# goalheart/ionic-mpnn

Measured on AMD Instinct MI355X. Metric: molecule-graph pairs/sec (fwd), batch 4096 per MI355X, higher is better.
Workload: dtype f32 (bf16x9 emulation)

## Files before the change

### ionic_mpnn_amd/csrc/encoder_typed.hip

```cpp
#include "encoder_device.h"
#include "encoder_layout.h"
#include "kernel_device.h"

namespace impnn {
namespace enc {

namespace {

constexpr int kOffUpd = 0;
constexpr int off_h(bool x3) { return kOffUpd + (x3 ? kXUpdLds : kTUpdLds); }
constexpr int kTHSBig3 = 32;
constexpr int off_msg(bool x3, int hs = kTHS) { return off_h(x3) + kRCap * hs; }
constexpr int off_rec(bool x3, int ecap, int hs = kTHS) { return off_msg(x3, hs) + tmsg_floats(ecap); }
constexpr size_t lds_fixed_bytes(bool x3, int Vb, int ecap, int hs = kTHS) {
  return sizeof(float) * (size_t)off_rec(x3, ecap, hs) + trec_lds_bytes(Vb, ecap);
}
static_assert(lds_fixed_bytes(true, kTVbMax, kTECap) <= 160 * 1024 && lds_fixed_bytes(false, kTVbMax, kTECapBig) <= 160 * 1024 &&
                  lds_fixed_bytes(true, kTVbMax, kTECapBig, kTHSBig3) <= 160 * 1024,
              "LDS budget");

typedef bf16x8_t bf16x8;
struct B3 {
  bf16x8 p0, p1, p2;
};
__device__ __forceinline__ B3 split8x3(f32x4 a, f32x4 b) {
  union {
    bf16x8 v;
    unsigned u[4];
  } q0, q1, q2;
  split_pair(a[0], a[1], q0.u[0], q1.u[0], q2.u[0]);
  split_pair(a[2], a[3], q0.u[1], q1.u[1], q2.u[1]);
  split_pair(b[0], b[1], q0.u[2], q1.u[2], q2.u[2]);
  split_pair(b[2], b[3], q0.u[3], q1.u[3], q2.u[3]);
  B3 r;
  r.p0 = q0.v;
  r.p1 = q1.v;
  r.p2 = q2.v;
  return r;
}
__device__ __forceinline__ void mma9x2(f32x4& c0, f32x4& c1, const __bf16* blk0, const __bf16* blk1, int lane, const B3& b) {
  const bf16x8 a00 = *reinterpret_cast<const bf16x8*>(blk0 + lane * 8);
  const bf16x8 a01 = *reinterpret_cast<const bf16x8*>(blk0 + 512 + lane * 8);
  const bf16x8 a02 = *reinterpret_cast<const bf16x8*>(blk0 + 1024 + lane * 8);
  const bf16x8 a10 = *reinterpret_cast<const bf16x8*>(blk1 + lane * 8);
  const bf16x8 a11 = *reinterpret_cast<const bf16x8*>(blk1 + 512 + lane * 8);
  const bf16x8 a12 = *reinterpret_cast<const bf16x8*>(blk1 + 1024 + lane * 8);
  c0 = mfma_bf16(a02, b.p2, c0);  c1 = mfma_bf16(a12, b.p2, c1);
  c0 = mfma_bf16(a01, b.p2, c0);  c1 = mfma_bf16(a11, b.p2, c1);
  c0 = mfma_bf16(a02, b.p1, c0);  c1 = mfma_bf16(a12, b.p1, c1);
  c0 = mfma_bf16(a00, b.p2, c0);  c1 = mfma_bf16(a10, b.p2, c1);
  c0 = mfma_bf16(a02, b.p0, c0);  c1 = mfma_bf16(a12, b.p0, c1);
  c0 = mfma_bf16(a01, b.p1, c0);  c1 = mfma_bf16(a11, b.p1, c1);
  c0 = mfma_bf16(a00, b.p1, c0);  c1 = mfma_bf16(a10, b.p1, c1);
  c0 = mfma_bf16(a01, b.p0, c0);  c1 = mfma_bf16(a11, b.p0, c1);
  c0 = mfma_bf16(a00, b.p0, c0);  c1 = mfma_bf16(a10, b.p0, c1);
}

template <int ABID>
__device__ __forceinline__ f32x4 mfma1(float a, float b, f32x4 c) {
  return __builtin_amdgcn_mfma_f32_4x4x1f32(a, b, c, 3, ABID, 0);
}

typedef float f32x2v __attribute__((ext_vector_type(2)));
typedef __attribute__((address_space(3))) void* lds_ptr_t;
__device__ __forceinline__ void glds16(const void* gsrc, const float* dst) {
  const unsigned lds_dst = __builtin_amdgcn_readfirstlane((unsigned)(uintptr_t)(lds_ptr_t)dst);
  unsigned keep;
  asm volatile("s_mov_b32 %0, m0\n\ts_mov_b32 m0, %2\n\ts_nop 0\n\tglobal_load_lds_dwordx4 %1, off\n\ts_mov_b32 m0, %0"
               : "=&s"(keep)
               : "v"(gsrc), "s"(lds_dst)
               : "memory");
}
struct Grp {
  uint4 ge;
  f32x2v aq;
};
struct Run {
  f32x4 bq[4];
  Grp first;
};

__device__ __forceinline__ void group_messages(const f32x2v aq, const f32x4 (&bq)[4], float& m01, float& m23) {
  f32x4 acc0 = {0.f, 0.f, 0.f, 0.f}, acc1 = acc0;
#ifndef IMPNN_DIAG_NO_MSG_MFMA
  acc0 = mfma1<0>(aq[0], bq[0][0], acc0);
  acc1 = mfma1<0>(aq[1], bq[0][1], acc1);
  acc0 = mfma1<1>(aq[0], bq[0][2], acc0);
  acc1 = mfma1<1>(aq[1], bq[0][3], acc1);
  acc0 = mfma1<2>(aq[0], bq[1][0], acc0);
  acc1 = mfma1<2>(aq[1], bq[1][1], acc1);
  acc0 = mfma1<3>(aq[0], bq[1][2], acc0);
  acc1 = mfma1<3>(aq[1], bq[1][3], acc1);
  acc0 = mfma1<4>(aq[0], bq[2][0], acc0);
  acc1 = mfma1<4>(aq[1], bq[2][1], acc1);
  acc0 = mfma1<5>(aq[0], bq[2][2], acc0);
  acc1 = mfma1<5>(aq[1], bq[2][3], acc1);
  acc0 = mfma1<6>(aq[0], bq[3][0], acc0);
  acc1 = mfma1<6>(aq[1], bq[3][1], acc1);
  acc0 = mfma1<7>(aq[0], bq[3][2], acc0);
  acc1 = mfma1<7>(aq[1], bq[3][3], acc1);
#else
  acc0[0] = aq[0] + bq[0][0] + bq[3][3];
  acc1[1] = aq[1] + bq[1][1] + bq[2][2];
#endif
  float x0 = acc0[0] + acc1[0], x1 = acc0[1] + acc1[1], x2 = acc0[2] + acc1[2], x3 = acc0[3] + acc1[3];
  asm volatile("s_nop 1\n\tv_permlane32_swap_b32 %0, %1\n\tv_permlane32_swap_b32 %2, %3"
               : "+v"(x0), "+v"(x1), "+v"(x2), "+v"(x3));
  m01 = x0 + x1;
  m23 = x2 + x3;
}

__global__ __launch_bounds__(256) void typed_m0_kernel(const float* tmat0, const float* atom_table, float* m0,
                                                       M0Header* hdr, int Va, int Vb, int S) {
  const int lane = threadIdx.x & 63;
  const int w = __builtin_amdgcn_readfirstlane(blockIdx.x * 4 + (threadIdx.x >> 6));
  const int nga = (Va + 4) >> 2;
  if (w < Vb * nga) {
    const int v = w / nga, a0 = 4 * (w - v * nga);
    const int kh = lane >> 5, f = lane & 31;
    const int ai = a0 + (lane & 3);
    f32x2v aq = {0.f, 0.f};
    if (ai < Va) aq = *reinterpret_cast<const f32x2v*>(atom_table + (size_t)ai * kD + 16 * kh + 2 * ((lane >> 2) & 7));
    const float* bp = tmat0 + (size_t)v * kTMatFloats + kh * 512 + f * 4;
    f32x4 bq[4];
#pragma unroll
    for (int i = 0; i < 4; ++i) bq[i] = ld4(bp + i * 128);
    float m01, m23;
    group_messages(aq, bq, m01, m23);
    float* row = m0 + (size_t)v * (Va + 1) * kD + f;
    if (a0 + kh <= Va) row[(size_t)(a0 + kh) * kD] = m01;
    if (a0 + 2 + kh <= Va) row[(size_t)(a0 + 2 + kh) * kD] = m23;
  }
  if (blockIdx.x == 0 && threadIdx.x == 0) *hdr = M0Header{kM0Magic, Va, Vb, S};
}

#ifndef IMPNN_T_PF
#define IMPNN_T_PF 0
#endif
#ifndef IMPNN_T_EARLY
#define IMPNN_T_EARLY 0
#endif
constexpr int kPfWhere = IMPNN_T_PF, kRunsEarly = IMPNN_T_EARLY;
template <int N, bool LANES>
__device__ __forceinline__ void reduce_ranks(const float* msg, const uint16_t* jdptr, int d0, int deg, int row, int q,
                                             int zero_slot, f32x4& agg0, f32x4& agg1) {
  const uint2 jd = *reinterpret_cast<const uint2*>(jdptr + d0);
  const int first[4] = {(int)(jd.x & 0xffffu), (int)(jd.x >> 16), (int)(jd.y & 0xffffu), (int)(jd.y >> 16)};
  f32x4 m0v[N], m1v[N];
#pragma unroll
  for (int j = 0; j < N; ++j) {
    const int o = tmsg_off(d0 + j < deg ? first[j] + row : zero_slot, q);
    m0v[j] = ld4(msg + o);
    m1v[j] = ld4(msg + (o ^ 16));
  }
#pragma unroll
  for (int j = 0; j < N; ++j) {
    if constexpr (LANES) {
#pragma unroll
      for (int i = 0; i < 4; ++i) {
        agg0[i] = lane1(agg0[i] + m0v[j][i]);
        agg1[i] = lane1(agg1[i] + m1v[j][i]);
      }
    } else {
      agg0 += m0v[j];
      agg1 += m1v[j];
    }
  }
}

__device__ __forceinline__ float keep1(float v) { return lane1(v); }
__device__ __forceinline__ f32x4 keep1(f32x4 v) { return v; }
template <bool LANES, class F, class... A>
__device__ __forceinline__ f32x4 quad(F f, A... a) {
  if constexpr (LANES) {
    f32x4 r;
#pragma unroll
    for (int i = 0; i < 4; ++i) r[i] = f(a[i]...);
    return r;
  } else {
    return f(a...);
  }
}

template <bool STAMPS, bool X3, int HS = kTHS>
__global__ __launch_bounds__(kThreads, kThreads / 256) void encoder_typed_kernel(TEncParams p) {
  extern __shared__ __align__(16) float smem[];
  constexpr int kUpdLds = X3 ? kXUpdLds : kTUpdLds, kUpdSlot = X3 ? kXUpdSlot : kTUpdSlot;
  constexpr int kNPf = X3 ? 3 : 2;
  float* const wupd = smem + kOffUpd;
  float* const wvec = wupd + (X3 ? kXVecFloatOff : kTVecFloatOff);
  float* const hbuf = smem + off_h(X3);
  float* const msg = smem + off_msg(X3, HS);
  const int zero_slot = p.ecap + 1;
  unsigned char* const recl = reinterpret_cast<unsigned char*>(smem + off_rec(X3, p.ecap, HS));
  const int rec_lds = p.rec_lds;
  float* const atab = reinterpret_cast<float*>(recl + rec_lds);
  const uint16_t* const r_rowdeg = reinterpret_cast<const uint16_t*>(recl + kTRecRowdeg);
  const unsigned char* const r_tilemax = recl + kTRecTilemax;
  const uint16_t* const r_moloff = reinterpret_cast<const uint16_t*>(recl + kTRecMoloff);
  const uint16_t* const r_molrows = reinterpret_cast<const uint16_t*>(recl + kTRecMolrows);
  const uint16_t* const r_poolrow = reinterpret_cast<const uint16_t*>(recl + kTRecPoolrow);
  const int32_t* const r_rowatom = reinterpret_cast<const int32_t*>(recl + kTRecRowatom);
  const uint16_t* const r_jdptr = reinterpret_cast<const uint16_t*>(recl + kTRecJdptr);
  const uint16_t* const r_runs = reinterpret_cast<const uint16_t*>(recl + trec_runs_off(p.Vb, p.ecap));
  int* const run_ctr = reinterpret_cast<int*>(recl + kTRecCounts + 8);
  const uint4* const r_grp = reinterpret_cast<const uint4*>(recl + kTRecGrp);

  const int tid = threadIdx.x, lane = tid & 63;
  const int wave = __builtin_amdgcn_readfirstlane(tid >> 6);
  const int a = lane & 15, q = lane >> 4;
  unsigned long long* stamp = STAMPS && p.stamps ? p.stamps + (size_t)blockIdx.x * 32 : nullptr;
  if (stamp && tid == 0) stamp[0] = __builtin_amdgcn_s_memtime();

  {
    const PlanHeader hd = *p.header;
    if (hd.magic != kPlanMagic || hd.kind != 1 || hd.nwg != (int)gridDim.x || hd.max_sub != p.max_sub ||
        hd.B != p.B || hd.n_ions != p.n_ions || hd.overflow != 0) {
      const float nan = __builtin_nanf("");
      for (int g = 0; g < p.n_ions; ++g)
        for (int64_t t = (int64_t)blockIdx.x * kThreads + tid; t < (int64_t)p.B * kD; t += (int64_t)gridDim.x * kThreads)
          p.pooled[g][t] = nan;
      return;
    }
  }
  const int c_begin = blockIdx.x * p.max_sub;
  const int c_end = c_begin + __builtin_amdgcn_readfirstlane(p.nsub[blockIdx.x]);
  if (c_begin >= c_end) return;

  if (p.atab_lds)
    for (int t = tid; t < (p.Va + 1) * (kTAS / 4); t += kThreads)
      st4(atab + 4 * t, t < p.Va * (kD / 4) ? ld4(p.atom_table + 4 * t) : f32x4{0.f, 0.f, 0.f, 0.f});
  if (tid < kD) msg[zero_slot * kD + tid] = 0.f;
  unsigned long long t_pro = 0, t_steps = 0, t_pool = 0, t_mark = 0, t_msg = 0;
  if (stamp && tid == 0) t_mark = __builtin_amdgcn_s_memtime();

  auto pool = [&](int M, int m0, int g) {
    float* out_g = p.pooled[g];
    for (int t0 = 0; t0 < M * 64; t0 += kThreads) {
      const int t = t0 + tid;
      const int part = t & 7, f4 = (t >> 3) & 7, m = t >> 6;
      f32x4 acc = {0.f, 0.f, 0.f, 0.f};
      if (m < M) {
        const int nr = r_molrows[m], mo = r_moloff[m];
        for (int n = part; n < nr; n += 8) {
          const int pr = r_poolrow[mo + n];
          if (pr & 0x8000) acc += ld4(hbuf + (pr & 0xff) * HS + 4 * f4);
        }
      }
#pragma unroll
      for (int i = 0; i < 4; ++i) {
        float v = acc[i];
        v += __builtin_bit_cast(float, __builtin_amdgcn_update_dpp(0, __builtin_bit_cast(int, v), 0xb1, 0xf, 0xf, true));
        v += __builtin_bit_cast(float, __builtin_amdgcn_update_dpp(0, __builtin_bit_cast(int, v), 0x4e, 0xf, 0xf, true));
        v += __builtin_bit_cast(float, __builtin_amdgcn_update_dpp(0, __builtin_bit_cast(int, v), 0x141, 0xf, 0xf, true));
        acc[i] = v;
      }
      if (m < M && part == 0) st4(out_g + (int64_t)(m0 + m) * kD + 4 * f4, acc);
    }
  };
  auto fill_h0 = [&]() {
    const int row = tid >> 2, sub = tid & 3;
    const int id = r_rowatom[row];
    f32x4 v0 = {0.f, 0.f, 0.f, 0.f}, v1 = v0;
    if ((unsigned)id < (unsigned)p.Va) {
      if (p.atab_lds) {
        v0 = ld4(atab + id * kTAS + 8 * sub);
        v1 = ld4(atab + id * kTAS + 8 * sub + 4);
      } else {
        int sb = sub;
        asm volatile("" : "+v"(sb));
        v0 = ld4(p.atom_table + (int64_t)id * kD + 8 * sb);
        v1 = ld4(p.atom_table + (int64_t)id * kD + 8 * sb + 4);
      }
    }
    st4(hbuf + row * HS + 8 * sub, v0);
    st4(hbuf + row * HS + 8 * sub + 4, v1);
  };

  if (p.S == 0) {
    for (int c = c_begin; c < c_end; ++c) {
      const unsigned char* rc = p.rec + (size_t)c * kTRecBytes;
      if (8 * tid < rec_lds) reinterpret_cast<uint2*>(recl)[tid] = reinterpret_cast<const uint2*>(rc)[tid];
      const int4 dsc = reinterpret_cast<const int4*>(p.desc)[c];
      lds_barrier();
      fill_h0();
      lds_barrier();
      pool(__builtin_amdgcn_readfirstlane(dsc.y), __builtin_amdgcn_readfirstlane(dsc.x),
           __builtin_amdgcn_readfirstlane(dsc.w) >> 16);
      lds_barrier();
    }
    return;
  }

  unsigned tabmask = 0;
  {
    const M0Header t0 = *reinterpret_cast<const M0Header*>(p.upd[0] + kUpdLds);
    if (t0.magic == kM0Magic && t0.Va == p.Va && t0.Vb == p.Vb && t0.S == p.S) tabmask |= 1u;
    if (p.n_ions > 1) {
      const M0Header t1 = *reinterpret_cast<const M0Header*>(p.upd[1] + kUpdLds);
      if (t1.magic == kM0Magic && t1.Va == p.Va && t1.Vb == p.Vb && t1.S == p.S) tabmask |= 2u;
    }
  }

  const bool rec_big = rec_lds > kTRecPart1;
  const unsigned char* rec_c = p.rec + (size_t)c_begin * kTRecBytes;
  uint2 rec_n8 = reinterpret_cast<const uint2*>(rec_c)[tid];
  uint32_t rec_n4 = rec_big ? reinterpret_cast<const uint32_t*>(rec_c + kTRecPart1)[tid] : 0u;
  int4 dsc_next = reinterpret_cast<const int4*>(p.desc)[c_begin];

  auto fetch_step0 = [&](const int4 dn, int cn) {
    const int gn = __builtin_amdgcn_readfirstlane(dn.w) >> 16;
    const float* const ug = p.upd[gn];
    static_assert(kUpdLds % 256 == 0, "whole 64-lane transfers");
    int ln = lane, wv = wave;
    asm volatile("" : "+v"(ln), "+s"(wv));
    const bool tabn = (tabmask >> gn) & 1u;
    int edges = __builtin_amdgcn_readfirstlane(dn.z);
    edges = tabn ? (edges < p.ecap ? edges : p.ecap) : 0;
    constexpr int kIt = (kTECapBig / 8 + kWaves - 1) / kWaves;
    uint32_t sw[kIt];
    if (tabn) {
      const uint32_t* const lst = p.slist + (size_t)cn * p.ecap;
#pragma unroll
      for (int i = 0; i < kIt; ++i) {
        const int sl = 8 * (wv + i * kWaves) + (ln >> 3);
        const uint32_t word = lst[sl < edges ? sl : 0];
        sw[i] = sl < edges ? word : 0u;
      }
    } else {
#pragma unroll
      for (int i = 0; i < kIt; ++i) sw[i] = 0u;
    }
    constexpr int kUIt = (kUpdLds / 256 + kWaves - 1) / kWaves;
#pragma unroll
    for (int i = 0; i < kUIt; ++i) {
      const int ub = 64 * (wv + i * kWaves);
      if (ub < kUpdLds / 4) glds16(ug + 4 * (ub + ln), wupd + 4 * ub);
    }
    static_assert(kIt == 5, "the list words are landed by name");
    asm volatile("" : "+v"(sw[0]), "+v"(sw[1]), "+v"(sw[2]), "+v"(sw[3]), "+v"(sw[4]) : : "memory");
    const float* const m0_g = p.m0[gn];
#pragma unroll
    for (int i = 0; i < kIt; ++i) {
      const int base = 8 * (wv + i * kWaves);
      if (base < edges) {
        const int sl = base + (ln >> 3);
        const unsigned type = min(sw[i] >> 24, (unsigned)p.Vb - 1u), col = min(sw[i] & kSrcIdNone, (unsigned)p.Va);
        const unsigned off = (type * (unsigned)(p.Va + 1) + col) * kD + 4u * ((ln & 7) ^ ((sl >> 1) & 7));
        glds16(m0_g + off, msg + kD * base);
      }
    }
  };
  fetch_step0(dsc_next, c_begin);

  const uint32_t* const grp_x = reinterpret_cast<const uint32_t*>(r_grp);
  const int kh = lane >> 5, f = lane & 31;
  const int boff = kh * 512 + f * 4;
  const int ysh = 8 * (lane & 3), zsh = 16 * kh;
  const int acol = 16 * kh + 2 * ((lane >> 2) & 7);

  for (int c = c_begin; c < c_end; ++c) {
    const int4 dsc = dsc_next;
    const int m0 = __builtin_amdgcn_readfirstlane(dsc.x), M = __builtin_amdgcn_readfirstlane(dsc.y);
    const int rg = __builtin_amdgcn_readfirstlane(dsc.w);
    const int R = rg & 0xffff, g = rg >> 16;
    const int ntiles = (R + 15) >> 4;
    const float* upd_g = p.upd[g];
    const float* tmat_g = p.tmat[g];
    const bool tab0 = (tabmask >> g) & 1u;
    if (8 * tid < rec_lds) reinterpret_cast<uint2*>(recl)[tid] = rec_n8;
    if (rec_big && kTRecPart1 + 4 * tid < rec_lds) reinterpret_cast<uint32_t*>(recl + kTRecPart1)[tid] = rec_n4;
    lds_barrier();
    fill_h0();
    if (tid == 0) *run_ctr = 2 * kWaves;
    asm volatile("s_waitcnt vmcnt(0) lgkmcnt(0)\n\ts_barrier" ::: "memory");
    {
      const int cn = (c + 1) < c_end ? (c + 1) : c;
      const unsigned char* rn = p.rec + (size_t)cn * kTRecBytes;
      rec_n8 = reinterpret_cast<const uint2*>(rn)[tid];
      if (rec_big) rec_n4 = reinterpret_cast<const uint32_t*>(rn + kTRecPart1)[tid];
      dsc_next = reinterpret_cast<const int4*>(p.desc)[cn];
    }
    if (stamp && tid == 0) {
      const unsigned long long t = __builtin_amdgcn_s_memtime();
      t_pro += t - t_mark;
      t_mark = t;
    }
    const int nrun = __builtin_amdgcn_readfirstlane(*reinterpret_cast<const uint16_t*>(recl + kTRecNrun));

    Run P, Q;
    int gP = 0, nP = 0, gQ = 0, nQ = 0;
    bool haveP = false, haveQ = false;
    const bool sP = wave < nrun, sQ = wave + kWaves < nrun;
    const int sgP = __builtin_amdgcn_readfirstlane(r_runs[sP ? wave : 0]);
    const int snP = __builtin_amdgcn_readfirstlane(r_runs[(sP ? wave : 0) + 1]) - sgP;
    const int sgQ = __builtin_amdgcn_readfirstlane(r_runs[sQ ? wave + kWaves : 0]);
    const int snQ = __builtin_amdgcn_readfirstlane(r_runs[(sQ ? wave + kWaves : 0) + 1]) - sgQ;
    const int soP = sP ? (__builtin_amdgcn_readfirstlane(grp_x[4 * sgP]) & 0xff) * kTMatFloats : 0;
    const int soQ = sQ ? (__builtin_amdgcn_readfirstlane(grp_x[4 * sgQ]) & 0xff) * kTMatFloats : 0;
    const int lboffP = sP ? boff : 0, lboffQ = sQ ? boff : 0;
    f32x4 pf[kNPf];
    auto fetch_pf = [&](int s_) {
#pragma unroll
      for (int i = 0; i < kNPf; ++i) pf[i] = ld4(upd_g + (int64_t)s_ * kUpdSlot + 4 * (tid + i * kThreads));
    };
    auto fetch_P = [&](int s_) {
      const float* tm = tmat_g + (size_t)s_ * p.Vb * kTMatFloats;
#pragma unroll
      for (int i = 0; i < 4; ++i) P.bq[i] = ld4(tm + soP + lboffP + i * 128);
    };
    auto fetch_Q = [&](int s_) {
      const float* tm = tmat_g + (size_t)s_ * p.Vb * kTMatFloats;
#pragma unroll
      for (int i = 0; i < 4; ++i) Q.bq[i] = ld4(tm + soQ + lboffQ + i * 128);
    };
    if (kRunsEarly >= 1) fetch_P(0);
    if (kRunsEarly >= 2) fetch_Q(0);
    if (stamp && c == c_begin && tid == 0) stamp[13] = __builtin_amdgcn_s_memtime();
    for (int s = 0; s < p.S; ++s) {
      const float* tm_s = tmat_g + (size_t)s * p.Vb * kTMatFloats;
      __builtin_amdgcn_s_setprio(2);
      const bool from_tab = tab0 && s == 0;
      if (kPfWhere == 0) {
        if (s > 0) {
          fetch_pf(s);
        } else {
#pragma unroll
          for (int i = 0; i < kNPf; ++i) pf[i] = f32x4{0.f, 0.f, 0.f, 0.f};
        }
      }
      if (!from_tab) {
        const float* const abase = hbuf + acol;
        auto load_group = [&](int e, Grp& G) {
          G.ge = r_grp[e];
          const int src = __builtin_amdgcn_ubfe(G.ge.y, ysh, 8);
          G.aq = *reinterpret_cast<const f32x2v*>(abase + src * HS);
        };
        auto compute = [&](const Grp& G, const f32x4 (&bq)[4]) {
          float m01, m23;
          group_messages(G.aq, bq, m01, m23);
          msg[__builtin_amdgcn_ubfe(G.ge.z, zsh, 16) ^ f] = m01;
          msg[__builtin_amdgcn_ubfe(G.ge.w, zsh, 16) ^ f] = m23;
        };
        auto run_type = [&](int g_, int n_, Run& Rn) {
          const int end = g_ + n_;
          Grp T;
          int e = g_;
          while (true) {
            if (e + 1 < end) load_group(e + 1, T);
            compute(Rn.first, Rn.bq);
            if (++e >= end) break;
            if (e + 1 < end) load_group(e + 1, Rn.first);
            compute(T, Rn.bq);
            if (++e >= end) break;
          }
        };
        auto fetch = [&](bool have, int r, int& g_, int& n_, Run& Rn, const float* tm) {
          const int rc = have ? r : 0;
          g_ = __builtin_amdgcn_readfirstlane(r_runs[rc]);
          n_ = __builtin_amdgcn_readfirstlane(r_runs[rc + 1]) - g_;
          const int type = have ? (__builtin_amdgcn_readfirstlane(grp_x[4 * g_]) & 0xff) : 0;
          const float* bp = tm + (size_t)type * kTMatFloats + (have ? boff : 0);
#pragma unroll
          for (int i = 0; i < 4; ++i) Rn.bq[i] = ld4(bp + i * 128);
        };
        auto next_run = [&]() {
          int r = 0;
          if (lane == 0) r = atomicAdd(run_ctr, 1);
          return __builtin_amdgcn_readfirstlane(r);
        };
        auto take = [&](int r, int& g_, int& n_, Run& Rn) {
          fetch(true, r, g_, n_, Rn, tm_s);
          load_group(g_, Rn.first);
        };
        auto landed = [](f32x4 (&b)[4]) {
          asm volatile("" : "+v"(b[0]), "+v"(b[1]), "+v"(b[2]), "+v"(b[3]) : : "memory");
        };
        if (kRunsEarly < 1) fetch_P(s);
        if (kRunsEarly < 2) fetch_Q(s);
        haveP = sP; gP = sgP; nP = snP;
        haveQ = sQ; gQ = sgQ; nQ = snQ;
        if (haveP) load_group(gP, P.first);
        if (haveQ) load_group(gQ, Q.first);
        if (haveP) {
          if (!haveQ) {
            landed(P.bq);
            run_type(gP, nP, P);
          } else {
            while (true) {
              landed(P.bq);
              run_type(gP, nP, P);
              const int rP = next_run();
              if (rP >= nrun) {
                landed(Q.bq);
                run_type(gQ, nQ, Q);
                break;
              }
              take(rP, gP, nP, P);
              landed(Q.bq);
              run_type(gQ, nQ, Q);
              const int rQ = next_run();
              if (rQ >= nrun) {
                landed(P.bq);
                run_type(gP, nP, P);
                break;
              }
              take(rQ, gQ, nQ, Q);
            }
          }
        }
        landed(P.bq);
        landed(Q.bq);
      }
      if (s > 0) {
#pragma unroll
        for (int i = 0; i < kNPf; ++i)
          if (4 * (tid + i * kThreads) < kUpdLds) st4(wupd + 4 * (tid + i * kThreads), pf[i]);
      }
      const bool mstamp = stamp && c == c_begin && s == 1;
      if (mstamp && lane == 0) stamp[16 + wave] = __builtin_amdgcn_s_memtime();
      lds_barrier();
      if (tid == 0) *run_ctr = 2 * kWaves;
      if (mstamp && tid == 0) stamp[12] = __builtin_amdgcn_s_memtime();
      if (stamp && tid == 0 && c == c_begin && s == 1) t_msg = __builtin_amdgcn_s_memtime();

      int my_tile = -1;
      {
        const int grp = wave & 3, slot = wave >> 2, q4 = ntiles >> 2, r4 = ntiles & 3;
        const int heavy = (4 - r4) * q4;
        if (grp >= r4) {
          if (slot < q4) my_tile = slot * (4 - r4) + (grp - r4);
        } else if (slot <= q4) {
          my_tile = heavy + slot * r4 + grp;
        }
      }
      const bool has_tile = my_tile >= 0 && my_tile < ntiles;
      if (has_tile) {
        const int tile = my_tile;
        const int row = tile * 16 + a;
        const int deg = r_rowdeg[row];
        const int maxdeg = __builtin_amdgcn_readfirstlane(r_tilemax[tile]);
        f32x4 h0, h1, z0, z1, r0, r1;
        [[maybe_unused]] const __bf16* const wb = reinterpret_cast<const __bf16*>(wupd);
        if constexpr (X3) {
          h0 = ld4(hbuf + row * HS + 4 * q);
          h1 = ld4(hbuf + row * HS + 16 + 4 * q);
          z0 = ld4(wvec + 0 * kD + 4 * q), z1 = ld4(wvec + 0 * kD + 16 + 4 * q);
          r0 = ld4(wvec + 1 * kD + 4 * q), r1 = ld4(wvec + 1 * kD + 16 + 4 * q);
          const B3 sh = split8x3(h0, h1);
          mma9x2(z0, z1, wb + ((0 * 2 + 0) * 2 + 0) * 1536, wb + ((0 * 2 + 1) * 2 + 0) * 1536, lane, sh);
          mma9x2(r0, r1, wb + ((1 * 2 + 0) * 2 + 0) * 1536, wb + ((1 * 2 + 1) * 2 + 0) * 1536, lane, sh);
        }
        f32x4 agg0 = {0.f, 0.f, 0.f, 0.f}, agg1 = agg0;
        if (maxdeg <= 2) {
          if (maxdeg == 1) reduce_ranks<1, X3>(msg, r_jdptr, 0, deg, row, q, zero_slot, agg0, agg1);
          if (maxdeg == 2) reduce_ranks<2, X3>(msg, r_jdptr, 0, deg, row, q, zero_slot, agg0, agg1);
        } else {
          for (int d0 = 0; d0 < maxdeg; d0 += 4) reduce_ranks<4, X3>(msg, r_jdptr, d0, deg, row, q, zero_slot, agg0, agg1);
        }
        if (mstamp && wave == 1 && lane == 0) stamp[8] = __builtin_amdgcn_s_memtime();
        __builtin_amdgcn_s_setprio(1);
        if (s + 1 < p.S) {
          if (kPfWhere == 1) fetch_pf(s + 1);
          if (kRunsEarly >= 1) fetch_P(s + 1);
          if (kRunsEarly >= 2) fetch_Q(s + 1);
        }
        if constexpr (!X3) {
          h0 = ld4(hbuf + row * HS + 4 * q);
          h1 = ld4(hbuf + row * HS + 16 + 4 * q);
          z0 = ld4(wvec + 0 * kD + 4 * q), z1 = ld4(wvec + 0 * kD + 16 + 4 * q);
          r0 = ld4(wvec + 1 * kD + 4 * q), r1 = ld4(wvec + 1 * kD + 16 + 4 * q);
        }
        f32x4 t0 = ld4(wvec + 2 * kD + 4 * q), t1 = ld4(wvec + 2 * kD + 16 + 4 * q);
        if constexpr (X3) {
          const B3 sa = split8x3(agg0, agg1);
          mma9x2(z0, z1, wb + ((0 * 2 + 0) * 2 + 1) * 1536, wb + ((0 * 2 + 1) * 2 + 1) * 1536, lane, sa);
          mma9x2(r0, r1, wb + ((1 * 2 + 0) * 2 + 1) * 1536, wb + ((1 * 2 + 1) * 2 + 1) * 1536, lane, sa);
          z0 = sigmoid4_lanes(z0);
          z1 = sigmoid4_lanes(z1);
          const f32x4 rh0 = mul4_lanes(sigmoid4_lanes(r0), h0);
          const f32x4 rh1 = mul4_lanes(sigmoid4_lanes(r1), h1);
          const B3 srh = split8x3(rh0, rh1);
          mma9x2(t0, t1, wb + ((2 * 2 + 0) * 2 + 0) * 1536, wb + ((2 * 2 + 1) * 2 + 0) * 1536, lane, srh);
          mma9x2(t0, t1, wb + ((2 * 2 + 0) * 2 + 1) * 1536, wb + ((2 * 2 + 1) * 2 + 1) * 1536, lane, sa);
        } else {
          const float* wl = wupd + 4 * lane;
#pragma unroll
          for (int half = 0; half < 2; ++half) {
#pragma unroll
            for (int u = 0; u < 2; ++u) {
              const int hu = half * 2 + u;
              const f32x4 Az0 = ld4(wl + ((0 * 2 + 0) * 4 + hu) * 256);
              const f32x4 Az1 = ld4(wl + ((0 * 2 + 1) * 4 + hu) * 256);
              const f32x4 Ar0 = ld4(wl + ((1 * 2 + 0) * 4 + hu) * 256);
              const f32x4 Ar1 = ld4(wl + ((1 * 2 + 1) * 4 + hu) * 256);
              const f32x4 Bv = half == 0 ? (u == 0 ? h0 : h1) : (u == 0 ? agg0 : agg1);
#pragma unroll
              for (int r = 0; r < 4; ++r) {
                z0 = mfma4(Az0[r], Bv[r], z0);
                z1 = mfma4(Az1[r], Bv[r], z1);
                r0 = mfma4(Ar0[r], Bv[r], r0);
                r1 = mfma4(Ar1[r], Bv[r], r1);
              }
            }
          }
          z0 = sigmoid4<false>(z0);
          z1 = sigmoid4<false>(z1);
          const f32x4 rh0 = sigmoid4<false>(r0) * h0;
          const f32x4 rh1 = sigmoid4<false>(r1) * h1;
#pragma unroll
          for (int half = 0; half < 2; ++half) {
#pragma unroll
            for (int u = 0; u < 2; ++u) {
              const int hu = half * 2 + u;
              const f32x4 Ah0 = ld4(wl + ((2 * 2 + 0) * 4 + hu) * 256);
              const f32x4 Ah1 = ld4(wl + ((2 * 2 + 1) * 4 + hu) * 256);
              const f32x4 Bv = half == 0 ? (u == 0 ? rh0 : rh1) : (u == 0 ? agg0 : agg1);
#pragma unroll
              for (int r = 0; r < 4; ++r) {
                t0 = mfma4(Ah0[r], Bv[r], t0);
                t1 = mfma4(Ah1[r], Bv[r], t1);
              }
            }
          }
        }
        __builtin_amdgcn_s_setprio(0);
        if (kPfWhere == 2 && s + 1 < p.S) {
          asm volatile("" ::: "memory");
          fetch_pf(s + 1);
        }
        if (mstamp && wave == 1 && lane == 0) stamp[9] = __builtin_amdgcn_s_memtime();
        const f32x4 gm0 = ld4(wvec + 3 * kD + 4 * q), gm1 = ld4(wvec + 3 * kD + 16 + 4 * q);
        const f32x4 bt0 = ld4(wvec + 4 * kD + 4 * q), bt1 = ld4(wvec + 4 * kD + 16 + 4 * q);
        __builtin_amdgcn_sched_barrier(0);
        const f32x4 th0 = X3 ? tanh4_lanes(t0) : tanh4<false>(t0), th1 = X3 ? tanh4_lanes(t1) : tanh4<false>(t1);
        const auto blend = [](auto z, auto th, auto h) { return keep1(z * (th - h) + h); };
        f32x4 n0 = quad<X3>(blend, z0, th0, h0), n1 = quad<X3>(blend, z1, th1, h1);
        const f32x4 s4 = quad<X3>([](auto x, auto y) { return keep1(x + y); }, n0, n1);
        const float sum = sum_xor16_xor32((s4[0] + s4[1]) + (s4[2] + s4[3]));
        const float mean = sum * (1.0f / kD);
        const auto center = [mean](auto n) { return keep1(n - mean); };
        n0 = quad<X3>(center, n0);
        n1 = quad<X3>(center, n1);
        const f32x4 q4 = quad<X3>([](auto x, auto y) { return keep1(x * x + y * y); }, n0, n1);
        const float var = sum_xor16_xor32((q4[0] + q4[1]) + (q4[2] + q4[3]));
        const float inv = __builtin_amdgcn_rsqf(var * (1.0f / kD) + p.ln_eps);
        const auto affine = [inv](auto n, auto gm, auto bt, auto h) { return keep1(n * keep1(gm * inv) + keep1(bt + h)); };
        const f32x4 o0 = quad<X3>(affine, n0, gm0, bt0, h0), o1 = quad<X3>(affine, n1, gm1, bt1, h1);
        st4(hbuf + row * HS + 4 * q, o0);
        st4(hbuf + row * HS + 16 + 4 * q, o1);
        if (mstamp && wave == 1 && lane == 0) stamp[10] = __builtin_amdgcn_s_memtime();
      }
      if (!has_tile && s + 1 < p.S) {
        if (kPfWhere != 0) fetch_pf(s + 1);
        if (kRunsEarly >= 1) fetch_P(s + 1);
        if (kRunsEarly >= 2) fetch_Q(s + 1);
      }
      if (mstamp && wave == 1 && lane == 0) stamp[11] = __builtin_amdgcn_s_memtime();
      lds_barrier();
      if (stamp && c == c_begin && s < 2 && tid == 0) stamp[14 + s] = __builtin_amdgcn_s_memtime();
    }
    if (stamp && tid == 0) {
      const unsigned long long t = __builtin_amdgcn_s_memtime();
      t_steps += t - t_mark;
      t_mark = t;
    }

    asm volatile(""
                 : "+v"(rec_n8.x), "+v"(rec_n8.y), "+v"(rec_n4), "+v"(dsc_next.x), "+v"(dsc_next.y), "+v"(dsc_next.z),
                   "+v"(dsc_next.w)
                 :
                 : "memory");
    if (c + 1 < c_end) fetch_step0(dsc_next, c + 1);
    pool(M, m0, g);
    lds_barrier();
    if (stamp && tid == 0) {
      const unsigned long long t = __builtin_amdgcn_s_memtime();
      t_pool += t - t_mark;
      t_mark = t;
    }
  }
  if (stamp && tid == 0) {
    stamp[1] = t_pro;
    stamp[2] = t_steps;
    stamp[3] = t_pool;
    stamp[4] = (unsigned long long)(c_end - c_begin);
    stamp[5] = t_msg;
    stamp[7] = __builtin_amdgcn_s_memtime();
  }
}

}
}

bool encoder_typed_supported(int N, int E, int D, int S, int Vb) {
  using namespace enc;
  if (D != kD || S < 0) return false;
  if (N < 1 || N > 0xffff || E < 0 || E > 0xffff) return false;
  if (Vb < 1 || Vb > kTVbMax) return false;
  return true;
}

size_t encoder_typed_prepared_bytes(int S, int Vb, bool x3) {
  return enc::typed_prepared_floats(S, Vb, x3) * sizeof(float);
}

int launch_encoder_typed_prepare(const float* weights, const float* bond_table, int K, int S, int Vb, bool x3,
                                 void* prepared, hipStream_t s) {
  if (S <= 0) return IMPNN_OK;
  enc::TImageParams ip{};
  ip.weights = weights;
  ip.bond_table = bond_table;
  ip.prepared = static_cast<float*>(prepared);
  ip.K = K;
  ip.S = S;
  ip.Vb = Vb;
  ip.x3 = x3 ? 1 : 0;
  ip.step_floats = impnn_encoder_step_floats(enc::kD, K);
  return enc::launch_typed_image(ip, s);
}

size_t encoder_typed_prepared_bytes_atoms(int S, int Va, int Vb, bool x3) {
  return (enc::typed_prepared_floats(S, Vb, x3) + enc::m0_table_floats(S, Va, Vb)) * sizeof(float);
}

int launch_encoder_typed_prepare_atoms(const float* weights, const float* bond_table, const float* atom_table, int Va,
                                       int K, int S, int Vb, bool x3, void* prepared, hipStream_t s) {
  using namespace enc;
  if (int rc = launch_encoder_typed_prepare(weights, bond_table, K, S, Vb, x3, prepared, s)) return rc;
  if (m0_table_floats(S, Va, Vb) == 0) return IMPNN_OK;
  float* img = static_cast<float*>(prepared);
  const size_t uslot = x3 ? kXUpdSlot : kTUpdSlot;
  const int waves = Vb * ((Va + 4) >> 2);
  typed_m0_kernel<<<(waves + 3) / 4, 256, 0, s>>>(img + (size_t)S * uslot, atom_table, img + typed_prepared_floats(S, Vb, x3),
                                                  reinterpret_cast<M0Header*>(img + (x3 ? kXUpdLds : kTUpdLds)), Va, Vb, S);
  return check_launch("typed_m0");
}

int launch_encoder_typed_run(const EncoderArgs& a, const enc::Ws& w, hipStream_t s) {
  using namespace enc;
  char* base = static_cast<char*>(a.workspace);
  TEncParams ep{};
  const size_t S1 = a.S > 0 ? a.S : 1;
  const bool x3 = a.mode == 3;
  const size_t uslot = x3 ? kXUpdSlot : kTUpdSlot;
  for (int g = 0; g < a.n_ions; ++g) {
    const float* prep;
    if (a.prepared[g]) {
      if (!aligned16(a.prepared[g])) return fail(IMPNN_E_BADARG, "encoder_fused: prepared weights must be 16B aligned");
      prep = static_cast<const float*>(a.prepared[g]);
    } else {
      float* img = reinterpret_cast<float*>(base + w.img_off) + (size_t)g * typed_prepared_floats(a.S, a.Vb, x3);
      if (int rc = launch_encoder_typed_prepare(a.weights[g], a.bond_table, a.K, a.S, a.Vb, x3, img, s)) return rc;
      prep = img;
    }
    ep.upd[g] = prep;
    ep.tmat[g] = prep + S1 * uslot;
    ep.m0[g] = prep + typed_prepared_floats(a.S, a.Vb, x3);
    ep.pooled[g] = a.pooled[g];
  }
  ep.atom_table = a.atom_table;
  ep.nsub = reinterpret_cast<const int32_t*>(base + w.nsub_off);
  ep.desc = reinterpret_cast<const int32_t*>(base + w.desc_off);
  ep.rec = reinterpret_cast<const unsigned char*>(base + w.rec_off);
  ep.slist = reinterpret_cast<const uint32_t*>(base + w.slist_off);
  ep.header = reinterpret_cast<const PlanHeader*>(base);
  ep.n_ions = a.n_ions; ep.B = a.B; ep.S = a.S; ep.Va = a.Va; ep.Vb = a.Vb; ep.max_sub = w.max_sub;
  ep.ln_eps = a.ln_eps;
  ep.stamps = nullptr;
  {
    size_t sb = 0;
    void* sp = debug_stamp_buffer(&sb);
    if (sp && sb >= (size_t)w.nwg * 32 * sizeof(unsigned long long)) ep.stamps = static_cast<unsigned long long*>(sp);
  }
  ep.upd_slot = (int)uslot;
  ep.ecap = tecap_of(a.E);
  ep.rec_lds = trec_lds_bytes(a.Vb, ep.ecap);
  const bool big3 = x3 && ep.ecap == kTECapBig;
  void (*kern)(TEncParams) =
      big3 ? (ep.stamps ? encoder_typed_kernel<true, true, kTHSBig3> : encoder_typed_kernel<false, true, kTHSBig3>)
      : x3 ? (ep.stamps ? encoder_typed_kernel<true, true> : encoder_typed_kernel<false, true>)
           : (ep.stamps ? encoder_typed_kernel<true, false> : encoder_typed_kernel<false, false>);
  if (int rc = ensure_lds_limit((const void*)kern, big3 ? (ep.stamps ? 10 : 9) : (ep.stamps ? 5 : 4) + (x3 ? 2 : 0))) return rc;
  size_t lds = lds_fixed_bytes(x3, a.Vb, ep.ecap, big3 ? kTHSBig3 : kTHS);
  const size_t atab_bytes = ((size_t)a.Va + 1) * kTAS * sizeof(float);
  ep.atab_lds = lds + atab_bytes <= 160 * 1024;
  if (ep.atab_lds) lds += atab_bytes;
  profile_record_start(s);
  kern<<<w.nwg, kThreads, lds, s>>>(ep);
  profile_record_stop(s);
  return check_launch("encoder_typed");
}

}
```

Before: 40.94 million.

## Split GRU weight staging into halves and overlap h-side MFMAs with message phase

Reorders the X3 update-weight LDS layout so the h-side gate blocks (part A) are contiguous and can be fetched separately via direct global-to-LDS loads. Part A for the next step is fetched right after the barrier, and part B during the current step, replacing the register-staged prefetch plus LDS store. The h-side z/r MFMAs now run before the aggregation barrier, overlapping the message phase, and a fused 4-accumulator MFMA routine interleaves them. Tile assignment is hoisted out of the step loop. This adds extra vmcnt waits and layout complexity, and it risks LDS hazards if the remapping is wrong.

```diff
diff --git a/ionic_mpnn_amd/csrc/encoder_typed.hip b/ionic_mpnn_amd/csrc/encoder_typed.hip
--- a/ionic_mpnn_amd/csrc/encoder_typed.hip
+++ b/ionic_mpnn_amd/csrc/encoder_typed.hip
@@ -18,6 +18,47 @@
 static_assert(lds_fixed_bytes(true, kTVbMax, kTECap) <= 160 * 1024 && lds_fixed_bytes(false, kTVbMax, kTECapBig) <= 160 * 1024 &&
                   lds_fixed_bytes(true, kTVbMax, kTECapBig, kTHSBig3) <= 160 * 1024,
               "LDS budget");
+
+constexpr int kXBlk = 3 * 512 / 2;
+constexpr int kXPartA = 4 * kXBlk + 2 * kD;
+constexpr int kXUnitsA = (kXPartA + 255) / 256;
+constexpr int kXUnitsB = (kXUpdLds - kXPartA + 255) / 256;
+static_assert(kXVecFloatOff == 12 * kXBlk && kXPartA + 8 * kXBlk == kXVecFloatOff + 2 * kD, "bh, gamma, beta stay in place");
+static_assert(kXPartA % 4 == 0 && kXPartA >= 256 && kXUpdLds - kXPartA >= 256 && kTUpdLds % 256 == 0, "whole units");
+constexpr int xlds_block(int blk) {
+  return blk < 8 && !(blk & 1) ? (blk >> 1) * kXBlk : kXPartA + (blk < 8 ? blk >> 1 : blk - 4) * kXBlk;
+}
+constexpr int xlds_vec(int v) { return v < 2 ? 4 * kXBlk + v * kD : kXVecFloatOff + v * kD; }
+constexpr int upd_units(bool x3, bool part_a) { return x3 ? (part_a ? kXUnitsA : kXUnitsB) : (part_a ? 0 : kTUpdLds / 256); }
+__device__ __forceinline__ int upd_unit_lds(bool x3, bool part_a, int k) {
+  if (!x3) return 256 * k;
+  if (part_a) return k < kXUnitsA - 1 ? 256 * k : kXPartA - 256;
+  return k < kXUnitsB - 1 ? kXPartA + 256 * k : kXUpdLds - 256;
+}
+__device__ __forceinline__ int upd_unit_src(bool x3, bool part_a, int k, int ln) {
+  if (!x3) return 256 * k + 4 * ln;
+  const int j = k / 3;
+  if (part_a) {
+    if (k < kXUnitsA - 1) return 256 * k + j * kXBlk + 4 * ln;
+    constexpr int tail = (kXPartA - 256) + 3 * kXBlk, lanes = (4 * kXBlk - (kXPartA - 256)) / 4;
+    return 4 * ln + (ln < lanes ? tail : kXVecFloatOff - 4 * lanes);
+  }
+  if (k < kXUnitsB - 1) return 256 * k + (j < 4 ? j + 1 : 4) * kXBlk + 4 * ln;
+  constexpr int lanes = (kXVecFloatOff + 2 * kD - (kXUpdLds - 256)) / 4;
+  return 4 * ln + (ln < lanes ? kXUpdLds - 256 - 2 * kD : kXUpdLds - 256);
+}
+constexpr int xlds_src(int x) {
+  if (x < 4 * kXBlk) return x + (x / kXBlk) * kXBlk;
+  if (x < kXPartA) return kXVecFloatOff + (x - 4 * kXBlk);
+  if (x < kXVecFloatOff + 2 * kD) return (x - kXPartA) + (((x - kXPartA) / kXBlk) < 4 ? (x - kXPartA) / kXBlk + 1 : 4) * kXBlk;
+  return x;
+}
+static_assert(xlds_src(xlds_block(0)) == 0 && xlds_src(xlds_block(6) + kXBlk - 4) == 7 * kXBlk - 4 &&
+                  xlds_src(xlds_block(1)) == kXBlk && xlds_src(xlds_block(7) + 4) == 7 * kXBlk + 4 &&
+                  xlds_src(xlds_block(8)) == 8 * kXBlk && xlds_src(xlds_block(11) + kXBlk - 4) == 12 * kXBlk - 4 &&
+                  xlds_src(xlds_vec(0)) == kXVecFloatOff && xlds_src(xlds_vec(1) + 28) == kXVecFloatOff + kD + 28 &&
+                  xlds_src(xlds_vec(2)) == kXVecFloatOff + 2 * kD && xlds_src(kXUpdLds - 4) == kXUpdLds - 4,
+              "mode 3: LDS order against slot order");
 
 typedef bf16x8_t bf16x8;
 struct B3 {
@@ -56,6 +97,25 @@
   c0 = mfma_bf16(a00, b.p0, c0);  c1 = mfma_bf16(a10, b.p0, c1);
 }
 
+__device__ __forceinline__ void mma9x4(f32x4& c0, f32x4& c1, f32x4& d0, f32x4& d1, const __bf16* blkc0, const __bf16* blkc1,
+                                       const __bf16* blkd0, const __bf16* blkd1, int lane, const B3& b) {
+  const __bf16* const blk[4] = {blkc0, blkc1, blkd0, blkd1};
+  bf16x8 w[4][3];
+#pragma unroll
+  for (int g = 0; g < 4; ++g)
+#pragma unroll
+    for (int pl = 0; pl < 3; ++pl) w[g][pl] = *reinterpret_cast<const bf16x8*>(blk[g] + 512 * pl + lane * 8);
+  f32x4* const acc[4] = {&c0, &c1, &d0, &d1};
+  constexpr int order[9][2] = {{2, 2}, {1, 2}, {2, 1}, {0, 2}, {2, 0}, {1, 1}, {0, 1}, {1, 0}, {0, 0}};
+#pragma unroll
+  for (int t = 0; t < 9; ++t)
+#pragma unroll
+    for (int g = 0; g < 4; ++g) {
+      const bf16x8 bt = order[t][1] == 0 ? b.p0 : order[t][1] == 1 ? b.p1 : b.p2;
+      *acc[g] = mfma_bf16(w[g][order[t][0]], bt, *acc[g]);
+    }
+}
+
 template <int ABID>
 __device__ __forceinline__ f32x4 mfma1(float a, float b, f32x4 c) {
   return __builtin_amdgcn_mfma_f32_4x4x1f32(a, b, c, 3, ABID, 0);
@@ -63,13 +123,16 @@
 
 typedef float f32x2v __attribute__((ext_vector_type(2)));
 typedef __attribute__((address_space(3))) void* lds_ptr_t;
-__device__ __forceinline__ void glds16(const void* gsrc, const float* dst) {
-  const unsigned lds_dst = __builtin_amdgcn_readfirstlane((unsigned)(uintptr_t)(lds_ptr_t)dst);
+__device__ __forceinline__ void glds16_at(const void* gsrc, unsigned lds_addr) {
+  const unsigned lds_dst = __builtin_amdgcn_readfirstlane(lds_addr);
   unsigned keep;
   asm volatile("s_mov_b32 %0, m0\n\ts_mov_b32 m0, %2\n\ts_nop 0\n\tglobal_load_lds_dwordx4 %1, off\n\ts_mov_b32 m0, %0"
                : "=&s"(keep)
                : "v"(gsrc), "s"(lds_dst)
                : "memory");
+}
+__device__ __forceinline__ void glds16(const void* gsrc, const float* dst) {
+  glds16_at(gsrc, (unsigned)(uintptr_t)(lds_ptr_t)dst);
 }
 struct Grp {
   uint4 ge;
@@ -134,13 +197,20 @@
   if (blockIdx.x == 0 && threadIdx.x == 0) *hdr = M0Header{kM0Magic, Va, Vb, S};
 }
 
-#ifndef IMPNN_T_PF
-#define IMPNN_T_PF 0
-#endif
 #ifndef IMPNN_T_EARLY
 #define IMPNN_T_EARLY 0
 #endif
-constexpr int kPfWhere = IMPNN_T_PF, kRunsEarly = IMPNN_T_EARLY;
+#ifndef IMPNN_T_HALVES
+#define IMPNN_T_HALVES 1
+#endif
+#ifndef IMPNN_T_HPRIO
+#define IMPNN_T_HPRIO 0
+#endif
+#ifndef IMPNN_T_H4
+#define IMPNN_T_H4 1
+#endif
+constexpr int kRunsEarly = IMPNN_T_EARLY, kHalves = IMPNN_T_HALVES, kHalvesPrio = IMPNN_T_HPRIO;
+constexpr bool kHalves4 = IMPNN_T_H4 != 0 && kHalves == 1;
 template <int N, bool LANES>
 __device__ __forceinline__ void reduce_ranks(const float* msg, const uint16_t* jdptr, int d0, int deg, int row, int q,
                                              int zero_slot, f32x4& agg0, f32x4& agg1) {
@@ -186,9 +256,9 @@
 __global__ __launch_bounds__(kThreads, kThreads / 256) void encoder_typed_kernel(TEncParams p) {
   extern __shared__ __align__(16) float smem[];
   constexpr int kUpdLds = X3 ? kXUpdLds : kTUpdLds, kUpdSlot = X3 ? kXUpdSlot : kTUpdSlot;
-  constexpr int kNPf = X3 ? 3 : 2;
   float* const wupd = smem + kOffUpd;
-  float* const wvec = wupd + (X3 ? kXVecFloatOff : kTVecFloatOff);
+  constexpr auto vec_off = [](int v) { return X3 ? xlds_vec(v) : kTVecFloatOff + v * kD; };
+  [[maybe_unused]] constexpr auto xblk = [](int gate, int T, int half) { return 2 * xlds_block((gate * 2 + T) * 2 + half); };
   float* const hbuf = smem + off_h(X3);
   float* const msg = smem + off_msg(X3, HS);
   const int zero_slot = p.ecap + 1;
@@ -258,8 +328,8 @@
       if (m < M && part == 0) st4(out_g + (int64_t)(m0 + m) * kD + 4 * f4, acc);
     }
   };
-  auto fill_h0 = [&]() {
-    const int row = tid >> 2, sub = tid & 3;
+  auto fill_h0 = [&](int t_) {
+    const int row = t_ >> 2, sub = t_ & 3;
     const int id = r_rowatom[row];
     f32x4 v0 = {0.f, 0.f, 0.f, 0.f}, v1 = v0;
     if ((unsigned)id < (unsigned)p.Va) {
@@ -283,7 +353,7 @@
       if (8 * tid < rec_lds) reinterpret_cast<uint2*>(recl)[tid] = reinterpret_cast<const uint2*>(rc)[tid];
       const int4 dsc = reinterpret_cast<const int4*>(p.desc)[c];
       lds_barrier();
-      fill_h0();
+      fill_h0(tid);
       lds_barrier();
       pool(__builtin_amdgcn_readfirstlane(dsc.y), __builtin_amdgcn_readfirstlane(dsc.x),
            __builtin_amdgcn_readfirstlane(dsc.w) >> 16);
@@ -308,10 +378,21 @@
   uint32_t rec_n4 = rec_big ? reinterpret_cast<const uint32_t*>(rec_c + kTRecPart1)[tid] : 0u;
   int4 dsc_next = reinterpret_cast<const int4*>(p.desc)[c_begin];
 
+  static_assert(upd_units(X3, true) <= 2 * kWaves && upd_units(X3, false) <= 2 * kWaves, "two units per wave at most");
+  auto fetch_upd = [&](const float* img, bool part_a, int ln, int wv) {
+    asm volatile("" : "+v"(ln), "+s"(wv));
+    const unsigned wupd_lds = (unsigned)(uintptr_t)(lds_ptr_t)wupd;
+#pragma unroll
+    for (int i = 0; i < 2; ++i) {
+      const int k = wv + i * kWaves;
+      if (k < upd_units(X3, part_a)) {
+        glds16_at(img + upd_unit_src(X3, part_a, k, ln), wupd_lds + 4u * (unsigned)upd_unit_lds(X3, part_a, k));
+      }
+    }
+  };
   auto fetch_step0 = [&](const int4 dn, int cn) {
     const int gn = __builtin_amdgcn_readfirstlane(dn.w) >> 16;
     const float* const ug = p.upd[gn];
-    static_assert(kUpdLds % 256 == 0, "whole 64-lane transfers");
     int ln = lane, wv = wave;
     asm volatile("" : "+v"(ln), "+s"(wv));
     const bool tabn = (tabmask >> gn) & 1u;
@@ -331,12 +412,8 @@
 #pragma unroll
       for (int i = 0; i < kIt; ++i) sw[i] = 0u;
     }
-    constexpr int kUIt = (kUpdLds / 256 + kWaves - 1) / kWaves;
-#pragma unroll
-    for (int i = 0; i < kUIt; ++i) {
-      const int ub = 64 * (wv + i * kWaves);
-      if (ub < kUpdLds / 4) glds16(ug + 4 * (ub + ln), wupd + 4 * ub);
-    }
+    fetch_upd(ug, true, ln, wv);
+    fetch_upd(ug, false, ln, wv);
     static_assert(kIt == 5, "the list words are landed by name");
     asm volatile("" : "+v"(sw[0]), "+v"(sw[1]), "+v"(sw[2]), "+v"(sw[3]), "+v"(sw[4]) : : "memory");
     const float* const m0_g = p.m0[gn];
@@ -368,17 +445,19 @@
     const float* upd_g = p.upd[g];
     const float* tmat_g = p.tmat[g];
     const bool tab0 = (tabmask >> g) & 1u;
-    if (8 * tid < rec_lds) reinterpret_cast<uint2*>(recl)[tid] = rec_n8;
-    if (rec_big && kTRecPart1 + 4 * tid < rec_lds) reinterpret_cast<uint32_t*>(recl + kTRecPart1)[tid] = rec_n4;
+    int tp = tid;
+    asm volatile("" : "+v"(tp));
+    if (8 * tp < rec_lds) reinterpret_cast<uint2*>(recl)[tp] = rec_n8;
+    if (rec_big && kTRecPart1 + 4 * tp < rec_lds) reinterpret_cast<uint32_t*>(recl + kTRecPart1)[tp] = rec_n4;
     lds_barrier();
-    fill_h0();
+    fill_h0(tp);
     if (tid == 0) *run_ctr = 2 * kWaves;
     asm volatile("s_waitcnt vmcnt(0) lgkmcnt(0)\n\ts_barrier" ::: "memory");
     {
       const int cn = (c + 1) < c_end ? (c + 1) : c;
       const unsigned char* rn = p.rec + (size_t)cn * kTRecBytes;
-      rec_n8 = reinterpret_cast<const uint2*>(rn)[tid];
-      if (rec_big) rec_n4 = reinterpret_cast<const uint32_t*>(rn + kTRecPart1)[tid];
+      rec_n8 = reinterpret_cast<const uint2*>(rn)[tp];
+      if (rec_big) rec_n4 = reinterpret_cast<const uint32_t*>(rn + kTRecPart1)[tp];
       dsc_next = reinterpret_cast<const int4*>(p.desc)[cn];
     }
     if (stamp && tid == 0) {
@@ -399,11 +478,6 @@
     const int soP = sP ? (__builtin_amdgcn_readfirstlane(grp_x[4 * sgP]) & 0xff) * kTMatFloats : 0;
     const int soQ = sQ ? (__builtin_amdgcn_readfirstlane(grp_x[4 * sgQ]) & 0xff) * kTMatFloats : 0;
     const int lboffP = sP ? boff : 0, lboffQ = sQ ? boff : 0;
-    f32x4 pf[kNPf];
-    auto fetch_pf = [&](int s_) {
-#pragma unroll
-      for (int i = 0; i < kNPf; ++i) pf[i] = ld4(upd_g + (int64_t)s_ * kUpdSlot + 4 * (tid + i * kThreads));
-    };
     auto fetch_P = [&](int s_) {
       const float* tm = tmat_g + (size_t)s_ * p.Vb * kTMatFloats;
 #pragma unroll
@@ -416,18 +490,43 @@
     };
     if (kRunsEarly >= 1) fetch_P(0);
     if (kRunsEarly >= 2) fetch_Q(0);
+    int my_tile = -1;
+    {
+      const int grp = wave & 3, slot = wave >> 2, q4 = ntiles >> 2, r4 = ntiles & 3;
+      const int heavy = (4 - r4) * q4;
+      if (grp >= r4) {
+        if (slot < q4) my_tile = slot * (4 - r4) + (grp - r4);
+      } else if (slot <= q4) {
+        my_tile = heavy + slot * r4 + grp;
+      }
+    }
+    const bool has_tile = my_tile >= 0 && my_tile < ntiles;
     if (stamp && c == c_begin && tid == 0) stamp[13] = __builtin_amdgcn_s_memtime();
     for (int s = 0; s < p.S; ++s) {
       const float* tm_s = tmat_g + (size_t)s * p.Vb * kTMatFloats;
+      const int row = (has_tile ? my_tile : 0) * 16 + a;
+      f32x4 h0, h1, z0, z1, r0, r1;
+      [[maybe_unused]] const __bf16* const wb = reinterpret_cast<const __bf16*>(wupd);
+      [[maybe_unused]] auto h_halves = [&]() {
+        if (has_tile) {
+          h0 = ld4(hbuf + row * HS + 4 * q);
+          h1 = ld4(hbuf + row * HS + 16 + 4 * q);
+          z0 = ld4(wupd + vec_off(0) + 4 * q), z1 = ld4(wupd + vec_off(0) + 16 + 4 * q);
+          r0 = ld4(wupd + vec_off(1) + 4 * q), r1 = ld4(wupd + vec_off(1) + 16 + 4 * q);
+          const B3 sh = split8x3(h0, h1);
+          if (kHalves4) {
+            mma9x4(z0, z1, r0, r1, wb + xblk(0, 0, 0), wb + xblk(0, 1, 0), wb + xblk(1, 0, 0), wb + xblk(1, 1, 0), lane, sh);
+          } else {
+            mma9x2(z0, z1, wb + xblk(0, 0, 0), wb + xblk(0, 1, 0), lane, sh);
+            mma9x2(r0, r1, wb + xblk(1, 0, 0), wb + xblk(1, 1, 0), lane, sh);
+          }
+        }
+      };
       __builtin_amdgcn_s_setprio(2);
       const bool from_tab = tab0 && s == 0;
-      if (kPfWhere == 0) {
-        if (s > 0) {
-          fetch_pf(s);
-        } else {
-#pragma unroll
-          for (int i = 0; i < kNPf; ++i) pf[i] = f32x4{0.f, 0.f, 0.f, 0.f};
-        }
+      if (s > 0) {
+        if (X3 && kHalves == 0) fetch_upd(upd_g + (int64_t)s * kUpdSlot, true, lane, wave);
+        fetch_upd(upd_g + (int64_t)s * kUpdSlot, false, lane, wave);
       }
       if (!from_tab) {
         const float* const abase = hbuf + acol;
@@ -482,6 +581,9 @@
         haveQ = sQ; gQ = sgQ; nQ = snQ;
         if (haveP) load_group(gP, P.first);
         if (haveQ) load_group(gQ, Q.first);
+        if constexpr (X3) {
+          if (kHalves == 2) h_halves();
+        }
         if (haveP) {
           if (!haveQ) {
             landed(P.bq);
@@ -512,44 +614,36 @@
         landed(P.bq);
         landed(Q.bq);
       }
-      if (s > 0) {
-#pragma unroll
-        for (int i = 0; i < kNPf; ++i)
-          if (4 * (tid + i * kThreads) < kUpdLds) st4(wupd + 4 * (tid + i * kThreads), pf[i]);
-      }
       const bool mstamp = stamp && c == c_begin && s == 1;
       if (mstamp && lane == 0) stamp[16 + wave] = __builtin_amdgcn_s_memtime();
+      if constexpr (X3) {
+        if (kHalves == 1 || (kHalves == 2 && from_tab)) {
+          __builtin_amdgcn_s_setprio(kHalvesPrio);
+          h_halves();
+        }
+        if (mstamp && wave == 1 && lane == 0) stamp[6] = __builtin_amdgcn_s_memtime();
+      }
+      if (s > 0) asm volatile("s_waitcnt vmcnt(0)" ::: "memory");
       lds_barrier();
+      if constexpr (X3 && kHalves != 0) {
+        if (s + 1 < p.S) fetch_upd(upd_g + (int64_t)(s + 1) * kUpdSlot, true, lane, wave);
+        __builtin_amdgcn_s_setprio(2);
+      }
       if (tid == 0) *run_ctr = 2 * kWaves;
       if (mstamp && tid == 0) stamp[12] = __builtin_amdgcn_s_memtime();
       if (stamp && tid == 0 && c == c_begin && s == 1) t_msg = __builtin_amdgcn_s_memtime();
 
-      int my_tile = -1;
-      {
-        const int grp = wave & 3, slot = wave >> 2, q4 = ntiles >> 2, r4 = ntiles & 3;
-        const int heavy = (4 - r4) * q4;
-        if (grp >= r4) {
-          if (slot < q4) my_tile = slot * (4 - r4) + (grp - r4);
-        } else if (slot <= q4) {
-          my_tile = heavy + slot * r4 + grp;
-        }
-      }
-      const bool has_tile = my_tile >= 0 && my_tile < ntiles;
       if (has_tile) {
         const int tile = my_tile;
-        const int row = tile * 16 + a;
         const int deg = r_rowdeg[row];
         const int maxdeg = __builtin_amdgcn_readfirstlane(r_tilemax[tile]);
-        f32x4 h0, h1, z0, z1, r0, r1;
-        [[maybe_unused]] const __bf16* const wb = reinterpret_cast<const __bf16*>(wupd);
         if constexpr (X3) {
-          h0 = ld4(hbuf + row * HS + 4 * q);
-          h1 = ld4(hbuf + row * HS + 16 + 4 * q);
-          z0 = ld4(wvec + 0 * kD + 4 * q), z1 = ld4(wvec + 0 * kD + 16 + 4 * q);
-          r0 = ld4(wvec + 1 * kD + 4 * q), r1 = ld4(wvec + 1 * kD + 16 + 4 * q);
-          const B3 sh = split8x3(h0, h1);
-          mma9x2(z0, z1, wb + ((0 * 2 + 0) * 2 + 0) * 1536, wb + ((0 * 2 + 1) * 2 + 0) * 1536, lane, sh);
-          mma9x2(r0, r1, wb + ((1 * 2 + 0) * 2 + 0) * 1536, wb + ((1 * 2 + 1) * 2 + 0) * 1536, lane, sh);
+          if (kHalves == 0) {
+            h_halves();
+          } else {
+            h0 = ld4(hbuf + row * HS + 4 * q);
+            h1 = ld4(hbuf + row * HS + 16 + 4 * q);
+          }
         }
         f32x4 agg0 = {0.f, 0.f, 0.f, 0.f}, agg1 = agg0;
         if (maxdeg <= 2) {
@@ -561,28 +655,27 @@
         if (mstamp && wave == 1 && lane == 0) stamp[8] = __builtin_amdgcn_s_memtime();
         __builtin_amdgcn_s_setprio(1);
         if (s + 1 < p.S) {
-          if (kPfWhere == 1) fetch_pf(s + 1);
           if (kRunsEarly >= 1) fetch_P(s + 1);
           if (kRunsEarly >= 2) fetch_Q(s + 1);
         }
         if constexpr (!X3) {
           h0 = ld4(hbuf + row * HS + 4 * q);
           h1 = ld4(hbuf + row * HS + 16 + 4 * q);
-          z0 = ld4(wvec + 0 * kD + 4 * q), z1 = ld4(wvec + 0 * kD + 16 + 4 * q);
-          r0 = ld4(wvec + 1 * kD + 4 * q), r1 = ld4(wvec + 1 * kD + 16 + 4 * q);
-        }
-        f32x4 t0 = ld4(wvec + 2 * kD + 4 * q), t1 = ld4(wvec + 2 * kD + 16 + 4 * q);
+          z0 = ld4(wupd + vec_off(0) + 4 * q), z1 = ld4(wupd + vec_off(0) + 16 + 4 * q);
+          r0 = ld4(wupd + vec_off(1) + 4 * q), r1 = ld4(wupd + vec_off(1) + 16 + 4 * q);
+        }
+        f32x4 t0 = ld4(wupd + vec_off(2) + 4 * q), t1 = ld4(wupd + vec_off(2) + 16 + 4 * q);
         if constexpr (X3) {
           const B3 sa = split8x3(agg0, agg1);
-          mma9x2(z0, z1, wb + ((0 * 2 + 0) * 2 + 1) * 1536, wb + ((0 * 2 + 1) * 2 + 1) * 1536, lane, sa);
-          mma9x2(r0, r1, wb + ((1 * 2 + 0) * 2 + 1) * 1536, wb + ((1 * 2 + 1) * 2 + 1) * 1536, lane, sa);
+          mma9x2(z0, z1, wb + xblk(0, 0, 1), wb + xblk(0, 1, 1), lane, sa);
+          mma9x2(r0, r1, wb + xblk(1, 0, 1), wb + xblk(1, 1, 1), lane, sa);
           z0 = sigmoid4_lanes(z0);
           z1 = sigmoid4_lanes(z1);
           const f32x4 rh0 = mul4_lanes(sigmoid4_lanes(r0), h0);
           const f32x4 rh1 = mul4_lanes(sigmoid4_lanes(r1), h1);
           const B3 srh = split8x3(rh0, rh1);
-          mma9x2(t0, t1, wb + ((2 * 2 + 0) * 2 + 0) * 1536, wb + ((2 * 2 + 1) * 2 + 0) * 1536, lane, srh);
-          mma9x2(t0, t1, wb + ((2 * 2 + 0) * 2 + 1) * 1536, wb + ((2 * 2 + 1) * 2 + 1) * 1536, lane, sa);
+          mma9x2(t0, t1, wb + xblk(2, 0, 0), wb + xblk(2, 1, 0), lane, srh);
+          mma9x2(t0, t1, wb + xblk(2, 0, 1), wb + xblk(2, 1, 1), lane, sa);
         } else {
           const float* wl = wupd + 4 * lane;
 #pragma unroll
@@ -625,13 +718,9 @@
           }
         }
         __builtin_amdgcn_s_setprio(0);
-        if (kPfWhere == 2 && s + 1 < p.S) {
-          asm volatile("" ::: "memory");
-          fetch_pf(s + 1);
-        }
         if (mstamp && wave == 1 && lane == 0) stamp[9] = __builtin_amdgcn_s_memtime();
-        const f32x4 gm0 = ld4(wvec + 3 * kD + 4 * q), gm1 = ld4(wvec + 3 * kD + 16 + 4 * q);
-        const f32x4 bt0 = ld4(wvec + 4 * kD + 4 * q), bt1 = ld4(wvec + 4 * kD + 16 + 4 * q);
+        const f32x4 gm0 = ld4(wupd + vec_off(3) + 4 * q), gm1 = ld4(wupd + vec_off(3) + 16 + 4 * q);
+        const f32x4 bt0 = ld4(wupd + vec_off(4) + 4 * q), bt1 = ld4(wupd + vec_off(4) + 16 + 4 * q);
         __builtin_amdgcn_sched_barrier(0);
         const f32x4 th0 = X3 ? tanh4_lanes(t0) : tanh4<false>(t0), th1 = X3 ? tanh4_lanes(t1) : tanh4<false>(t1);
         const auto blend = [](auto z, auto th, auto h) { return keep1(z * (th - h) + h); };
@@ -652,11 +741,13 @@
         if (mstamp && wave == 1 && lane == 0) stamp[10] = __builtin_amdgcn_s_memtime();
       }
       if (!has_tile && s + 1 < p.S) {
-        if (kPfWhere != 0) fetch_pf(s + 1);
         if (kRunsEarly >= 1) fetch_P(s + 1);
         if (kRunsEarly >= 2) fetch_Q(s + 1);
       }
       if (mstamp && wave == 1 && lane == 0) stamp[11] = __builtin_amdgcn_s_memtime();
+      if constexpr (X3 && kHalves != 0) {
+        if (s + 1 < p.S) asm volatile("s_waitcnt vmcnt(0)" ::: "memory");
+      }
       lds_barrier();
       if (stamp && c == c_begin && s < 2 && tid == 0) stamp[14 + s] = __builtin_amdgcn_s_memtime();
     }
```

New measurement: 40.86 million. No clear change (-0.2%).
